# tigrazone/zig_raytracing_contest

Measured on AMD Instinct MI355X. Metric: Mrays/sec + wall-clock to output.png on contest config.json scene, higher is better.
Workload: dtype f32; 1 GPU; cfg3: contest stand-in (99480 tris, 553091 refs), 1920x1080, 256 spp, max_bounce 4, grid 128^3; global_batch=530841600, parallelism=tiles1, schedule=timed: default pass sets

## Files before the change

### include/zrt.h

```cpp
#ifndef ZRT_H
#define ZRT_H

#include <stddef.h>
#include <stdint.h>

#ifdef __cplusplus
extern "C" {
#endif

#define ZRT_ABI_VERSION 2

typedef enum zrt_status {
    ZRT_OK = 0,
    ZRT_ERR_INVALID_ARG = -1,
    ZRT_ERR_NO_DEVICE = -2,
    ZRT_ERR_HIP = -3,
    ZRT_ERR_OUT_OF_MEMORY = -4,
    ZRT_ERR_UNSUPPORTED = -5,
    ZRT_ERR_IO = -6,
    ZRT_ERR_PARSE = -7,
    ZRT_ERR_NOT_FOUND = -8,
    ZRT_ERR_CAMERA = -9,
} zrt_status;

// ... 46 lines not shown
    uint64_t seed;
    int32_t device;
    uint32_t rank;
    uint32_t num_ranks;
    uint32_t tile_size;
    uint32_t flags;
    uint32_t samples_per_pass;
    uint32_t num_devices;
    uint32_t _reserved0;
    const int32_t* devices;
} zrt_render_config;

#define ZRT_FLAG_COUNT_STATS  0x1u
#define ZRT_FLAG_LANE_WALK    0x2u
#define ZRT_FLAG_ONE_SET      0x10u
#define ZRT_FLAG_KERNEL_TIMES 0x20u
#define ZRT_FLAG_ESCAPE       0x40u
#define ZRT_FLAG_NO_ESCAPE    0x80u
#define ZRT_FLAG_FRUSTUM      0x100u
#define ZRT_FLAG_NO_FRUSTUM   0x200u
#define ZRT_FLAG_MT_EXACT     0x400u
#define ZRT_FLAG_RELEASE      0x800u
#define ZRT_FLAG_NO_RELEASE   0x1000u

typedef struct zrt_stats {
    uint64_t segments;
    uint64_t cells_visited;
    uint64_t triangle_tests;
    uint64_t hits;
    uint64_t samples;
    double render_ms;
    double trace_kernel_ms;
    uint32_t trace_launches;
    uint32_t _pad;
} zrt_stats;

const char* zrt_error_string(int status);
int zrt_abi_version(void);
int zrt_device_count(int* count);
int zrt_device_warmup(int device);

typedef struct zrt_geometry zrt_geometry;

int zrt_geometry_build(const float* positions, const float* normals, const float* texcoords,
                       const uint32_t* material, uint32_t num_triangles,
                       const uint32_t resolution[3], uint32_t num_threads, zrt_geometry** out);
// ... 120 lines not shown
```

### zig_raytracing_contest_amd/csrc/escape.h

```cpp
#pragma once
#include <stdint.h>

#include "zrt_math.h"

namespace zrt {

#ifndef ZRT_ESC_BINS
#define ZRT_ESC_BINS 8
#endif
constexpr uint32_t kEscBins = ZRT_ESC_BINS;
constexpr uint32_t kEscNBin = 6 * kEscBins * kEscBins;
constexpr uint32_t kEscWords = kEscNBin <= 128 ? 4 : (kEscNBin + 31) / 32;
constexpr double kEscEps = 1e-3;

ZHD uint32_t esc_dir_bin(v3 d) {
    const float ax = fabsf(d.x), ay = fabsf(d.y), az = fabsf(d.z);
    uint32_t a;
    float m, u, v;
#if defined(__HIP_DEVICE_COMPILE__)
#define ZRT_ESC_RCP(x) __builtin_amdgcn_rcpf(x)
#else
#define ZRT_ESC_RCP(x) (1.0f / (x))
#endif
    if (ax >= ay && ax >= az) { a = 0; m = d.x; const float r = ZRT_ESC_RCP(ax); u = d.y * r; v = d.z * r; }
// ... 163 lines not shown
            }
            if (first < 0) first = it;
            last = it;
            run = 0;
        } else {
            if (run == 0) gap_it = it;
            ++run;
        }
    }
    frustum_finish(q, first, last, fb);
    if (first >= 0 && best_len > 0.0) {
        const double ta = (best0 * q.ds) * q.dmax, tb = (best1 * q.ds) * q.dmin;
        float ga = (float)ta, gb = (float)tb;
        if ((double)ga < ta) ga = nextafterf(ga, kInf);
        if ((double)gb > tb) gb = nextafterf(gb, 0.0f);
        if (ga < gb) {
            fb.ga = ga;
            fb.gb = gb;
        }
    }
    return fb;
}

}
```

### zig_raytracing_contest_amd/csrc/render.hip

```cpp
#include <hip/hip_runtime.h>

#include <algorithm>
#include <cstdio>
#include <cstdlib>
#include <cstring>
#include <ctime>
#include <new>
#include <vector>

#include "zrt_internal.h"
#include "dda.h"
#include "escape.h"
#include "device_geometry.h"

using namespace zrt;

#define HIP_TRY(expr)                                                            \
    do {                                                                         \
        hipError_t _e = (expr);                                                  \
        if (_e != hipSuccess) {                                                  \
            if (getenv("ZRT_DEBUG"))                                             \
                fprintf(stderr, "zrt: %s failed: %s (%s:%d)\n", #expr,           \
                        hipGetErrorString(_e), __FILE__, __LINE__);              \
            return _e == hipErrorOutOfMemory ? ZRT_ERR_OUT_OF_MEMORY : ZRT_ERR_HIP; \
// ... 489 lines not shown
}

struct WfParams {
    TraceParams t;
    const float4* q_in;
    float4* q_out;
    float4* stk4;
    float2* stk2;
    float4* term;
    uint32_t T;
    uint32_t* fetch8;
    const uint32_t* n_in8;
    uint32_t* n_out8;
    float4* hit;
    uint32_t* fetch8s;
    const uint32_t* occx;
    uint32_t occx_words, occx_nbw, occx_moff, occx_nb0, occx_nb01;
    uint32_t occx_ldsw;
    uint32_t test_min;
    uint32_t refill_min;
    uint32_t rel_min;
    uint32_t rel_emin;
    const uint32_t* esc;
};

constexpr uint32_t kCtr = 32;

__device__ __forceinline__ uint32_t xcd_q0(uint32_t P, uint32_t g) {
    const uint32_t nblk = (P + 63u) >> 6;
    return min(P, (nblk * g / 8u) * 64u);
}

__device__ __forceinline__ uint32_t region_base(const WfParams& w, uint32_t g) { return w.t.S * xcd_q0(w.t.P, g); }

#ifdef ZRT_SWEEP
#define SHADE_STAMP(k, v) do { if (sp) { asm volatile("" :: "v"(v)); const uint64_t t_ = __builtin_amdgcn_s_memtime(); \
    const uint32_t n_ = (uint32_t)__popcll(__ballot(1)); \
    if (first_active_lane()) { sp[k] += t_ - sp[16]; sp[16] = t_; sp[8 + (k)] += n_; } } } while (0)
#else
#define SHADE_STAMP(k, v) do { (void)sp; } while (0)
#endif
struct TriRec {
    float4 d0, d1, d2, d3;
};
__device__ __forceinline__ TriRec tri_rec(const TraceParams& p, float t, uint32_t hidx) {
    TriRec r;
// ... 242 lines not shown
#define ZRT_PARK_CHUNK 256
#endif
constexpr uint32_t kParkChunk = ZRT_PARK_CHUNK;
#ifndef ZRT_PARK_LATE_DRAIN
#define ZRT_PARK_LATE_DRAIN 1
#endif
#ifndef ZRT_PARK_QPF
#define ZRT_PARK_QPF 0
#endif
#ifndef ZRT_PARK_ADAPT
#define ZRT_PARK_ADAPT 1
#endif
__device__ __forceinline__ void park_load_range(const TraceParams& p, uint32_t pc, uint32_t* rng) {
    const uint32_t* c = p.cell32 + 8ull * pc;
    const uint32_t m0 = __builtin_amdgcn_readfirstlane((uint32_t)(uintptr_t)rng);
    asm volatile("s_mov_b32 m0, %2\n\t"
                 "global_load_lds_dword %0, off\n\t"
                 "s_add_u32 m0, m0, 0x100\n\t"
                 "global_load_lds_dword %1, off"
                 :
                 : "v"(c), "v"(c + 1), "s"(m0)
                 : "memory");
}
__device__ __forceinline__ void park_load_cell(const TraceParams& p, uint32_t pc, uint32_t face, uint32_t* rng) {
    const uint32_t* c = p.cell32 + 8ull * pc;
    const uint32_t m0 = __builtin_amdgcn_readfirstlane((uint32_t)(uintptr_t)rng);
    asm volatile("s_mov_b32 m0, %3\n\t"
                 "global_load_lds_dword %0, off\n\t"
                 "s_add_u32 m0, m0, 0x100\n\t"
                 "global_load_lds_dword %1, off\n\t"
                 "s_add_u32 m0, m0, 0x100\n\t"
                 "global_load_lds_dword %2, off"
                 :
                 : "v"(c), "v"(c + 1), "v"(c + 2 + face), "s"(m0)
                 : "memory");
}

__device__ __forceinline__ void park_load_esc(const uint32_t* word, uint32_t* esc) {
    const uint32_t m0 = __builtin_amdgcn_readfirstlane((uint32_t)(uintptr_t)esc);
    asm volatile("s_mov_b32 m0, %1\n\t"
                 "global_load_lds_dword %0, off"
                 :
                 : "v"(word), "s"(m0)
                 : "memory");
}

struct ParkSlot {
    float4 o[64];
    float4 d[64];
    unsigned long long best[64];
    float2 uv[64];
    uint32_t mark[64];
};

__device__ __forceinline__ uint32_t wave_excl_sum(uint32_t x, uint32_t lane, uint32_t& total) {
    uint32_t s = x;
    s += (uint32_t)__builtin_amdgcn_update_dpp(0, (int)s, 0x111, 0xf, 0xf, true);
    s += (uint32_t)__builtin_amdgcn_update_dpp(0, (int)s, 0x112, 0xf, 0xf, true);
// ... 113 lines not shown
                    ce = min(base + chunk, lim);
                    cgrp = grp;
                }
                const uint32_t take = min((uint32_t)__popcll(idle), ce - cb);
                const uint32_t rank = (uint32_t)__popcll(idle & below);
                if (st == kIdle && rank < take) {
                    {
                        qi = ent_index<false>(w, cgrp, cb + rank);
                        {
                            const float4 qa = w.q_in[3ull * qi], qb = w.q_in[3ull * qi + 1];
                            o = mk(qa.x, qa.y, qa.z);
                            d = mk(qb.x, qb.y, qb.z);
                        }
                        {
                            nearest = kInf;
                            hu = hv = 0.0f;
                            hidx = 0;
                            W.o[lane] = make_float4(o.x, o.y, o.z, 0.0f);
                            W.d[lane] = make_float4(d.x, d.y, d.z, 0.0f);
                            Dda s0;
                            if (ZRT_FAST_QUOT ? dda_init_fq(p.bmin, p.bmax, p.res, p.cs, p.ics, p.cs_ok != 0u, o, d, s0)
                                              : dda_init(p.bmin, p.bmax, p.res, p.cs, o, d, s0)) {
                                ddav_from_t<PK_BM>(s0, gk, pk, s);
                                if (ESC) {
                                    const uint32_t bin = esc_dir_bin(d);
                                    eoff = (bin >> 5) * 4u;
                                    emask = w.esc && s0.neg < 8u ? 1u << (bin & 31u) : 0u;
                                    eb = ~0u;
                                    esc_slot[lane] = 0u;
                                }
                                if (occx_cell<PK_BM>(occx_mask(L, occx_brick<PK_BM>(w, s)), s, pk)) {
                                    park_load_range(p, s.pc, rng_slot);
                                    rng_slot[128 + lane] = ~0u;
                                    st = kPark;
                                } else {
                                    st = kWalk;
                                }
                            } else {
                                st = kDone;
                            }
                        }
                    }
                }
                PARK_STAMP(12);
                cb += take;
                loaded = loaded || take != 0u;
                idle = __ballot(st == kIdle);
            }
            if (ZRT_PARK_LATE_DRAIN && !loaded) __builtin_amdgcn_s_waitcnt(0x3f70);
#if ZRT_PARK_QPF
            if (ce > cb) {
                const uint32_t j = min(cb + lane, ce - 1u);
                park_load_esc(reinterpret_cast<const uint32_t*>(w.q_in + 3ull * ent_index<false>(w, cgrp, j)), qpf_slot);
            }
#endif
            PARK_STAMP(0);
// ... 541 lines not shown
        r.q[3ull * i + 1] = make_float4(d.x, d.y, d.z, __uint_as_float(1u));
        rest = !ray_fast(d);
    }
    const uint64_t m = __ballot(rest);
    if (m != 0ull && (threadIdx.x & 63u) == (uint32_t)__builtin_ctzll(m)) atomicAdd(&r.ctr[2], (uint32_t)__popcll(m));
}

__global__ __launch_bounds__(kBlock) void rays_out_kernel(const RayParams r) {
    const uint32_t i = blockIdx.x * kBlock + threadIdx.x;
    if (i >= r.n) return;
    const float4 h = r.w.hit[i];
    ray_store_hit(r.hits, i, h.x, h.y, h.z, __float_as_uint(h.w));
}

using RayFn = void (*)(const RayParams);
const RayFn kRaysWalkBM = (RayFn)rays_walk_kernel<false, true, true, false>;
const RayFn kRaysWalk = (RayFn)rays_walk_kernel<false, true, false, false>;
const RayFn kRaysWalkWide = (RayFn)rays_walk_kernel<false, false, false, false>;
const RayFn kRaysWalkExact = (RayFn)rays_walk_kernel<false, false, false, true>;
const RayFn kRaysWalkCount = (RayFn)rays_walk_kernel<true, false, false, true>;
constexpr uint64_t kTraceChunk = 1ull << 20;
constexpr uint64_t kTraceParkMin = 1ull << 19;
constexpr uint32_t kTraceFlags = ZRT_FLAG_COUNT_STATS | ZRT_FLAG_LANE_WALK | ZRT_FLAG_MT_EXACT | ZRT_FLAG_ESCAPE |
                                 ZRT_FLAG_NO_ESCAPE | ZRT_FLAG_RELEASE | ZRT_FLAG_NO_RELEASE | ZRT_TRACE_PARK;

TraceFn count_fn(uint32_t max_bounce) {
    if (max_bounce <= 4) return (TraceFn)trace_kernel<4>;
    if (max_bounce <= 8) return (TraceFn)trace_kernel<8>;
    if (max_bounce <= 16) return (TraceFn)trace_kernel<16>;
    if (max_bounce <= 32) return (TraceFn)trace_kernel<32>;
    return nullptr;
}

struct DeviceGuard {
    int prev = -1;
    explicit DeviceGuard(int dev) {
        if (hipGetDevice(&prev) != hipSuccess) prev = -1;
        if (dev >= 0) (void)hipSetDevice(dev);
    }
    ~DeviceGuard() {
        if (prev >= 0) (void)hipSetDevice(prev);
    }
};

template <typename T>
int grow(T** p, size_t* cap, size_t n) {
    if (*cap >= n && *p) return ZRT_OK;
// ... 31 lines not shown
    zrt_grid grid{};
    uint32_t ncells = 0, nrefs = 0, nmat = 0;
    uint2* d_cells = nullptr;
    PackK pk{};
    bool packed = false;
    uint32_t* d_cell32 = nullptr;
    float* d_pos = nullptr;
    float4* d_data = nullptr;
    DevMat* d_mats = nullptr;
    float* d_texels = nullptr;
    double* d_zig = nullptr;
    uint32_t* d_occ = nullptr;
    uint32_t occ_shift = 0, occ_nb[3] = {0, 0, 0}, occ_words = 0;
    uint32_t* d_occx = nullptr;
    unsigned long long* d_bmask = nullptr;
    uint32_t* d_esc = nullptr;
    uint32_t* d_sat = nullptr;
    float4* d_tlo = nullptr; size_t tlo_cap = 0;
    bool esc_on = false;
    double rel_frac = 0.0;
    bool rel_on = false;
    bool esc_tried = false;
    double esc_density = 0.0;
    uint32_t occx_words = 0, occx_nbw = 0, occx_moff = 0, occx_nb[3] = {0, 0, 0};
    bool occx_ok = false;
    bool mt_exact = false;
    uint32_t* d_pix = nullptr; size_t pix_cap = 0;
    float4* d_out = nullptr; size_t out_cap = 0;
    struct PassSet {
        hipStream_t stream = nullptr;
        float4* q0 = nullptr; size_t q0_cap = 0;
        float4* q1 = nullptr; size_t q1_cap = 0;
        float4* term = nullptr; size_t term_cap = 0;
        float4* stk4 = nullptr; size_t stk4_cap = 0;
        float2* stk2 = nullptr; size_t stk2_cap = 0;
        uint32_t* wfc = nullptr; size_t wfc_cap = 0;
        float4* hit = nullptr; size_t hit_cap = 0;
        hipEvent_t ev_join = nullptr;
    };
    PassSet set[kMaxPassSets];
    float4* d_acc = nullptr; size_t acc_cap = 0;
    uint8_t* d_rgb = nullptr; size_t rgb_cap = 0;
    float* d_lin = nullptr; size_t lin_cap = 0;
    float* d_rays = nullptr; size_t rays_cap = 0;
    uint32_t* d_hits = nullptr; size_t hits_cap = 0;
    std::vector<hipEvent_t> ev_pass;
// ... 103 lines not shown
    if (hipGetDeviceCount(&n) != hipSuccess || n <= 0) return ZRT_ERR_NO_DEVICE;
    const double t1 = StageClock::now_ms();
    if (device < 0) device = 0;
    if (device >= n) return ZRT_ERR_NO_DEVICE;
    DeviceGuard g(device);
    HIP_TRY(hipFree(nullptr));
    const double t2 = StageClock::now_ms();
    hipFuncAttributes fa;
    HIP_TRY(hipFuncGetAttributes(&fa, (const void*)resolve_kernel));
    const double t3 = StageClock::now_ms();
    const int rc = grid_build_warmup();
    if (timing)
        fprintf(stderr, "timing: warm-up: runtime init (hipGetDeviceCount) %.3f ms, device context %.3f ms, "
                "render.hip code object %.3f ms, grid_build.hip code object %.3f ms\n",
                t1 - t0, t2 - t1, t3 - t2, StageClock::now_ms() - t3);
    return rc;
}

extern "C" void zrt_context_destroy(zrt_context* c) {
    if (!c) return;
    DeviceGuard g(c->device);
    if (c->d_cell32) (void)hipFree(c->d_cell32);
    void* bufs[] = {c->d_cells, c->d_pos, c->d_data, c->d_mats, c->d_texels, c->d_zig, c->d_occ, c->d_occx, c->d_esc,
                    c->d_bmask, c->d_sat, c->d_tlo,
                    c->d_pix, c->d_out, c->d_acc, c->d_rgb, c->d_lin, c->d_rays, c->d_hits, c->d_counter, c->d_stats};
    for (void* b : bufs)
        if (b) (void)hipFree(b);
    for (zrt_context::PassSet& ps : c->set) {
        void* sb[] = {ps.q0, ps.q1, ps.term, ps.stk4, ps.stk2, ps.wfc, ps.hit};
        for (void* b : sb)
            if (b) (void)hipFree(b);
        if (ps.ev_join) (void)hipEventDestroy(ps.ev_join);
        if (ps.stream && ps.stream != c->stream) (void)hipStreamDestroy(ps.stream);
    }
    for (hipEvent_t e : c->ev_trace) (void)hipEventDestroy(e);
    for (hipEvent_t e : c->ev_pass) (void)hipEventDestroy(e);
    for (hipEvent_t e : c->ev_k) (void)hipEventDestroy(e);
    if (c->ev_fork) (void)hipEventDestroy(c->ev_fork);
    if (c->ev_begin) (void)hipEventDestroy(c->ev_begin);
    if (c->ev_end) (void)hipEventDestroy(c->ev_end);
    if (c->stream) (void)hipStreamDestroy(c->stream);
    delete c;
}

namespace {

__global__ __launch_bounds__(kBlock) void occx_mask_kernel(const uint2* __restrict__ cells, uint32_t r0, uint32_t r1,
// ... 136 lines not shown
    if (!pack_is_linear(r, c->pk)) HIP_TRY(hipMemsetAsync(c->d_cell32, 0, 32 * n, c->stream));
    hipLaunchKernelGGL(cell32_kernel, dim3(std::min<uint32_t>((c->ncells + kBlock - 1) / kBlock, 16384)), dim3(kBlock),
                       0, c->stream, c->d_cells, r[0], r[1], r[2], c->ncells, c->pk, c->d_pos,
                       c->d_cell32);
    HIP_TRY(hipGetLastError());
    {
        unsigned long long h[2] = {0, 0};
        unsigned long long* d = nullptr;
        HIP_TRY(hipMalloc((void**)&d, sizeof h));
        hipError_t e = hipMemsetAsync(d, 0, sizeof h, c->stream);
        if (e == hipSuccess) {
            hipLaunchKernelGGL(release_stat_kernel, dim3(std::min<uint64_t>((n + kBlock - 1) / kBlock, 4096)),
                               dim3(kBlock), 0, c->stream, (const uint32_t*)c->d_cell32, n, d);
            e = hipGetLastError();
        }
        if (e == hipSuccess) e = hipMemcpyAsync(h, d, sizeof h, hipMemcpyDeviceToHost, c->stream);
        if (e == hipSuccess) e = hipStreamSynchronize(c->stream);
        (void)hipFree(d);
        HIP_TRY(e);
        c->rel_frac = h[0] ? (double)h[1] / (double)h[0] : 0.0;
        c->rel_on = c->rel_frac >= kRelMinFrac;
    }
    HIP_TRY(hipStreamSynchronize(c->stream));
    return ZRT_OK;
}

static int context_counters(zrt_context* c) {
    StageClock sc;
    int rc = context_packed(c);
    if (rc != ZRT_OK) return rc;
    sc.mark(c, "cell records (cell32_kernel)");
    HIP_TRY(hipMalloc((void**)&c->d_counter, 64));
    HIP_TRY(hipMalloc((void**)&c->d_stats, 512));
    return ZRT_OK;
}

static int context_init(zrt_context* c, const zrt_scene* s) {
    int rc = context_base(c);
    if (rc != ZRT_OK) return rc;
    c->grid = s->grid;
    c->ncells = s->num_cells;
    c->nrefs = s->num_triangles;
    c->nmat = s->num_materials;
    c->mt_exact = needs_mt_exact(s->triangles_pos, 9ull * s->num_triangles, 9u, 3u, 0x1p62f);
    HIP_TRY(hipMalloc((void**)&c->d_cells, 8ull * c->ncells));
    HIP_TRY(copy_sync(c->d_cells, s->cells, 8ull * c->ncells, hipMemcpyHostToDevice, c->stream));
// ... 547 lines not shown
        c->pix.resize(std::max<uint32_t>(n, 1));
        tile_pixels(key[0], key[1], key[2], key[3], key[4], c->pix.data(), &n);
        c->pix.resize(n);
        int r2 = grow(&c->d_pix, &c->pix_cap, std::max<size_t>(n, 1));
        if (r2 != ZRT_OK) return r2;
        if (n) HIP_TRY(copy_sync(c->d_pix, c->pix.data(), n * sizeof(uint32_t), hipMemcpyHostToDevice, c->stream));
        memcpy(c->pix_key, key, sizeof key);
        c->pix_valid = true;
    }
    const uint32_t P = (uint32_t)c->pix.size();
    zrt_stats st{};
    if (P == 0) { if (stats) *stats = st; return ZRT_OK; }

    const uint32_t spp = cfg->num_samples;
    const uint32_t mb = cfg->max_bounce;
    const uint32_t nb = std::max<uint32_t>(mb, 1);
    const uint64_t per_item = counting ? 16ull : 96ull + 16ull + 16ull + (ZRT_PLANES16 ? 32ull : 24ull) * nb;
    const bool big = (uint64_t)P * cfg->num_samples >= kSetsMinSamples;
    uint32_t want_sets = big ? kPassSets : 1u;
#if defined(ZRT_SWEEP) || defined(ZRT_SETS_ENV)
    if (const char* e = getenv("ZRT_SETS")) want_sets = (uint32_t)std::max(1, std::min((int)kMaxPassSets, atoi(e)));
#endif
    const bool ktimes = (cfg->flags & ZRT_FLAG_KERNEL_TIMES) != 0;
    size_t held = 16ull * c->out_cap;
    for (const zrt_context::PassSet& ps : c->set)
        held += 16ull * (ps.q0_cap + ps.q1_cap + ps.term_cap + ps.stk4_cap + ps.hit_cap) + 8ull * ps.stk2_cap +
                4ull * ps.wfc_cap;
    const uint64_t s_pass = pass_samples(cfg, per_item, P, counting ? 1u : want_sets, held, c->mem_share);
    const uint32_t npasses = (uint32_t)((spp + s_pass - 1) / s_pass);
    const uint32_t plan_sets = counting ? 1u : std::min<uint32_t>(npasses, want_sets);
    const uint32_t nsets = (cfg->flags & ZRT_FLAG_ONE_SET) ? 1u : plan_sets;
    uint32_t lead_pct = plan_sets > 1 ? kLeadPct : 0u;
#if defined(ZRT_SWEEP) || defined(ZRT_SETS_ENV)
    if (const char* e = getenv("ZRT_LEAD")) lead_pct = plan_sets > 1 ? (uint32_t)std::max(0, std::min(50, atoi(e))) : 0u;
#endif
    const uint64_t last_n = spp - (uint64_t)(npasses - 1) * s_pass;
    const uint64_t cap_items = std::max<uint64_t>(1, 0x7FFFFF00ull / P);
    const uint32_t lead = npasses > 1 ? (uint32_t)std::min<uint64_t>(
                                            {s_pass * lead_pct / 100, last_n - 1, cap_items - std::min(cap_items, s_pass)})
                                      : 0u;
    auto pass_first = [&](uint32_t pass) -> uint32_t { return pass == 0 ? 0u : (uint32_t)(pass * s_pass + lead); };
    auto pass_count = [&](uint32_t pass) -> uint32_t {
        return pass == 0 ? (uint32_t)std::min<uint64_t>(spp, s_pass + lead)
                         : (uint32_t)std::min<uint64_t>(s_pass, spp - pass_first(pass));
    };
    const uint64_t T = (s_pass + lead) * P;
    int rc;
// ... 44 lines not shown
    const bool park_next = c->occx_ok && !counting && !(cfg->flags & ZRT_FLAG_LANE_WALK) &&
                           c->packed && !mtx;
    const bool rel = !(cfg->flags & ZRT_FLAG_NO_RELEASE) && (c->rel_on || (cfg->flags & ZRT_FLAG_RELEASE));
    uint32_t test_min = rel ? kParkTestMinRel : kParkTestMin, refill_min = kParkRefillMin;
#if defined(ZRT_SWEEP) || defined(ZRT_SETS_ENV)
    if (const char* e = getenv("ZRT_PARK_T")) test_min = (uint32_t)std::max(1, std::min(64, atoi(e)));
    if (const char* e = getenv("ZRT_PARK_R")) refill_min = (uint32_t)std::max(1, std::min(64, atoi(e)));
#endif
    uint32_t rel_min = test_min;
    uint32_t rel_emin = 1;
#if defined(ZRT_SWEEP) || defined(ZRT_SETS_ENV)
    if (const char* e = getenv("ZRT_PARK_REL")) rel_min = (uint32_t)std::max(1, std::min(64, atoi(e)));
    if (const char* e = getenv("ZRT_PARK_REL_E")) rel_emin = (uint32_t)std::max(1, std::min(64, atoi(e)));
#endif
    const bool packed = c->packed && !mtx;
    const bool pbm = packed && c->pk.bm;
    const WfFn f_first = mtx ? kWfPrimaryExact : packed ? (pbm ? kWfPrimaryBM : kWfPrimary) : kWfPrimaryWide;
    if (!c->esc_tried && park_next && !(cfg->flags & ZRT_FLAG_NO_ESCAPE) && (big || (cfg->flags & ZRT_FLAG_ESCAPE))) {
        c->esc_tried = true;
        if ((rc = context_escape(c)) != ZRT_OK) return rc;
    }
    const bool esc = c->d_esc && !(cfg->flags & ZRT_FLAG_NO_ESCAPE) &&
                     (c->esc_on || (cfg->flags & ZRT_FLAG_ESCAPE));
    const WfFn f_next = park_next ? (pbm ? (esc ? (WfFn)wf_park_kernel<true, true> : (WfFn)wf_park_kernel<false, true>)
                                         : (esc ? (WfFn)wf_park_kernel<true, false> : (WfFn)wf_park_kernel<false, false>))
                                  : mtx ? kWfBounceExact : (packed ? (pbm ? kWfBounceBM : kWfBounce) : kWfBounceWide);
    const WfFn s_next = c->nmat <= kLdsMats ? (WfFn)wf_shade_kernel<true> : (WfFn)wf_shade_kernel<false>;
    const WfFn s_last = !ZRT_SHADE_LAST ? s_next
                        : c->nmat <= kLdsMats ? (WfFn)wf_shade_kernel<true, true> : (WfFn)wf_shade_kernel<false, true>;
    const size_t lds_shade = c->nmat <= kLdsMats ? c->nmat * sizeof(DevMat) : 0;
    for (uint32_t k = 0; k < nsets && park_next; ++k)
        if ((rc = grow(&c->set[k].hit, &c->set[k].hit_cap, T)) != ZRT_OK) return rc;

    {
        auto shortfall = [&](const char* what, const void* ptr, size_t cap, uint64_t need) {
            if (ptr && cap >= need) return false;
            if (getenv("ZRT_DEBUG"))
                fprintf(stderr, "zrt: capacity guard: %s holds %zu, the launch writes %llu\n", what, ptr ? cap : 0,
                        (unsigned long long)need);
            return true;
        };
        bool bad = shortfall("pixel list", c->d_pix, c->pix_cap, P) || shortfall("rgb", c->d_rgb, c->rgb_cap, 3ull * P) ||
                   (npasses > 1 && shortfall("accumulator", c->d_acc, c->acc_cap, P)) ||
                   (want_lin && shortfall("linear", c->d_lin, c->lin_cap, 3ull * P)) ||
                   (counting && shortfall("counting output", c->d_out, c->out_cap, T));
        for (uint32_t k = 0; k < nsets && !counting && !bad; ++k) {
// ... 133 lines not shown
        tp.sdiv = div_magic(S);
        const int first = pass == 0 ? 1 : 0, last = pass + 1 == npasses ? 1 : 0;
        if (!counting) {
            HIP_TRY(hipMemsetAsync(wfc, 0, 4ull * 32 * kCtr * (mb + 2), sm));
            WfParams W;
            memset(&W, 0, sizeof W);
            W.t = tp;
            W.stk4 = stk4;
            W.stk2 = stk2;
            W.term = term;
            W.T = (uint32_t)T;
            W.occx = c->d_occx;
            W.occx_words = c->occx_words;
            W.occx_ldsw = occx_ldsw;
            W.occx_nbw = c->occx_nbw;
            W.occx_moff = c->occx_moff;
            W.occx_nb0 = c->occx_nb[0];
            W.occx_nb01 = c->occx_nb[0] * c->occx_nb[1];
            W.test_min = test_min;
            W.refill_min = refill_min;
            W.rel_min = rel ? rel_min : 0u;
            W.rel_emin = rel_emin;
            W.esc = c->d_esc;
            for (uint32_t k = 0; k < nb; ++k) {
                W.q_in = (k & 1) ? q0 : q1;
                W.q_out = (k & 1) ? q1 : q0;
                W.fetch8 = wfc + kCtr * (16 * k);
                W.n_in8 = wfc + kCtr * (16 * k + 8);
                W.n_out8 = wfc + kCtr * (16 * (k + 1) + 8);
                W.hit = hit;
                W.fetch8s = wfc + kCtr * (16 * (mb + 2) + 8 * k);
                HIP_TRY(hipEventRecord(c->ev_trace[ne++], sm));
                const int cls = k == 0 ? ZRT_KERNEL_PRIMARY : (park_next ? ZRT_KERNEL_PARK : ZRT_KERNEL_BOUNCE);
                if ((rc = kt_begin(cls, sm)) != ZRT_OK) return rc;
                if (k == 0)
                    hipLaunchKernelGGL(f_first, dim3(grid_first), dim3(thr_first), lds_first, sm, W);
                else
                    hipLaunchKernelGGL(f_next, dim3(grid_next), dim3(thr_next), lds_next, sm, W);
                HIP_TRY(hipGetLastError());
                if ((rc = kt_end(sm)) != ZRT_OK) return rc;
                ++kp.launches[cls];
                if (k > 0 && park_next) {
                    if ((rc = kt_begin(ZRT_KERNEL_SHADE, sm)) != ZRT_OK) return rc;
                    if (k + 1 == nb)
                        hipLaunchKernelGGL(s_last, dim3(grid_shade_last), dim3(kTraceThreads), lds_shade, sm, W);
                    else
// ... 133 lines not shown

extern "C" int zrt_context_trace(zrt_context* c, const zrt_ray_batch* b, zrt_stats* stats) {
    if (!c || !b) return ZRT_ERR_INVALID_ARG;
    if ((b->flags & ~kTraceFlags) != 0u || b->on_device > 1u) return ZRT_ERR_INVALID_ARG;
    zrt_stats st{};
    if (b->num_rays == 0) { if (stats) *stats = st; return ZRT_OK; }
    if (!b->rays || !b->hits) return ZRT_ERR_INVALID_ARG;
    DeviceGuard g(c->device);

    const bool counting = (b->flags & ZRT_FLAG_COUNT_STATS) != 0;
    const bool mtx = c->mt_exact || (b->flags & ZRT_FLAG_MT_EXACT);
    const bool park_ok = c->occx_ok && !counting && !(b->flags & ZRT_FLAG_LANE_WALK) && c->packed && !mtx;
    const bool park = park_ok && ((b->flags & ZRT_TRACE_PARK) || b->num_rays >= kTraceParkMin);
    const bool packed = c->packed && !mtx;
    const bool pbm = packed && c->pk.bm;
    const bool rel = !(b->flags & ZRT_FLAG_NO_RELEASE) && (c->rel_on || (b->flags & ZRT_FLAG_RELEASE));
    int rc;
    if (!c->esc_tried && park && !(b->flags & ZRT_FLAG_NO_ESCAPE) &&
        (b->num_rays >= kSetsMinSamples || (b->flags & ZRT_FLAG_ESCAPE))) {
        c->esc_tried = true;
        if ((rc = context_escape(c)) != ZRT_OK) return rc;
    }
    const bool esc = c->d_esc && !(b->flags & ZRT_FLAG_NO_ESCAPE) && (c->esc_on || (b->flags & ZRT_FLAG_ESCAPE));
    const RayFn f_fast = (counting || mtx) ? nullptr : packed ? (pbm ? kRaysWalkBM : kRaysWalk) : kRaysWalkWide;
    const RayFn f_exact = counting ? kRaysWalkCount : kRaysWalkExact;
    const WfFn f_park = pbm ? (esc ? (WfFn)wf_park_kernel<true, true> : (WfFn)wf_park_kernel<false, true>)
                            : (esc ? (WfFn)wf_park_kernel<true, false> : (WfFn)wf_park_kernel<false, false>);

    zrt_context::PassSet& ps = c->set[0];
    const uint64_t per_ray = (b->on_device ? 0ull : 40ull) + (park ? 64ull : 0ull);
    const size_t held = 4ull * (c->rays_cap + c->hits_cap) + 16ull * (ps.q0_cap + ps.hit_cap);
    size_t budget = (size_t)144 << 30;
    size_t free_b = 0, total_b = 0;
    if (hipMemGetInfo(&free_b, &total_b) == hipSuccess && free_b) budget = std::min(budget, (free_b + held) / 10 * 6);
    budget /= std::max<uint32_t>(c->mem_share, 1u);
    uint64_t chunk = std::min<uint64_t>(kTraceChunk, b->num_rays);
    if (per_ray) chunk = std::max<uint64_t>(64, std::min<uint64_t>(chunk, budget / per_ray));
    if (!b->on_device) {
        if ((rc = grow(&c->d_rays, &c->rays_cap, 6 * chunk)) != ZRT_OK) return rc;
        if ((rc = grow(&c->d_hits, &c->hits_cap, 4 * chunk)) != ZRT_OK) return rc;
    }
    const size_t wfc_words = 32ull * kCtr * 2;
    if (park) {
        if ((rc = grow(&ps.q0, &ps.q0_cap, 3 * chunk)) != ZRT_OK) return rc;
        if ((rc = grow(&ps.hit, &ps.hit_cap, chunk)) != ZRT_OK) return rc;
        if ((rc = grow(&ps.wfc, &ps.wfc_cap, wfc_words)) != ZRT_OK) return rc;
    }
    if ((!b->on_device && (!c->d_rays || c->rays_cap < 6 * chunk || !c->d_hits || c->hits_cap < 4 * chunk)) ||
        (park && (!ps.q0 || ps.q0_cap < 3 * chunk || !ps.hit || ps.hit_cap < chunk || !ps.wfc ||
                  ps.wfc_cap < wfc_words)))
        return ZRT_ERR_INVALID_ARG;
    while (c->ev_trace.size() < 2) {
        hipEvent_t e;
        HIP_TRY(hipEventCreate(&e));
// ... 13 lines not shown
    memset(&R, 0, sizeof R);
    scene_params(c, R.w.t);
    R.w.t.max_bounce = 1;
    R.w.t.counter = c->d_counter;
    R.w.t.stats = c->d_stats;
    R.ctr = c->d_counter;
    if (park) {
        R.w.q_in = ps.q0;
        R.w.hit = ps.hit;
        R.w.fetch8 = ps.wfc;
        R.w.n_in8 = ps.wfc + 8 * kCtr;
        R.w.occx = c->d_occx;
        R.w.occx_words = c->occx_words;
        R.w.occx_ldsw = occx_ldsw;
        R.w.occx_nbw = c->occx_nbw;
        R.w.occx_moff = c->occx_moff;
        R.w.occx_nb0 = c->occx_nb[0];
        R.w.occx_nb01 = c->occx_nb[0] * c->occx_nb[1];
        R.w.test_min = rel ? kParkTestMinRel : kParkTestMin;
        R.w.refill_min = kParkRefillMin;
        R.w.rel_min = rel ? R.w.test_min : 0u;
        R.w.rel_emin = 1;
        R.w.esc = c->d_esc;
        R.q = ps.q0;
        R.n_in8 = ps.wfc + 8 * kCtr;
    }

    HIP_TRY(hipMemsetAsync(c->d_stats, 0, 512, c->stream));
    HIP_TRY(hipEventRecord(c->ev_begin, c->stream));
    uint32_t launches = 0;
    for (uint64_t off = 0; off < b->num_rays; off += chunk) {
        const uint32_t n = (uint32_t)std::min<uint64_t>(chunk, b->num_rays - off);
        if (b->on_device) {
            R.rays = b->rays + 6 * off;
            R.hits = reinterpret_cast<uint32_t*>(b->hits + off);
        } else {
            HIP_TRY(hipMemcpyAsync(c->d_rays, b->rays + 6 * off, 24ull * n, hipMemcpyHostToDevice, c->stream));
            R.rays = c->d_rays;
            R.hits = c->d_hits;
            HIP_TRY(hipEventRecord(c->ev_trace[0], c->stream));
        }
        R.n = n;
        HIP_TRY(hipMemsetAsync(c->d_counter, 0, 64, c->stream));
        const uint32_t nblk = (n + kBlock - 1) / kBlock;
        if (park) {
            HIP_TRY(hipMemsetAsync(ps.wfc, 0, 4ull * 16 * kCtr, c->stream));
// ... 209 lines not shown
            break;
        }
        case ZRT_PROBE_QUOT: {
            const float* a = (const float*)in + 2ull * i;
            float* o = (float*)out + 2ull * i;
            o[0] = quot_rn(a[0], a[1], mt_inv_det<false>(a[1]));
            o[1] = a[0] / a[1];
            break;
        }
        case ZRT_PROBE_RECIP: {
            const float x = ((const float*)in)[i];
            float* o = (float*)out + 2ull * i;
            o[0] = mt_inv_det<false>(x);
            o[1] = mt_inv_det<true>(x);
            break;
        }
        default:
            break;
    }
}

__global__ __launch_bounds__(kBlock) void recip_sweep_kernel(uint32_t lo, uint32_t count, uint32_t* out) {
    uint32_t bad = 0, first = 0xFFFFFFFFu;
    for (uint32_t k = blockIdx.x * kBlock + threadIdx.x; k < count; k += gridDim.x * kBlock) {
        const float x = __uint_as_float(lo + k);
        const float a = mt_inv_det<false>(x), b = mt_inv_det<true>(x);
        const bool same = __float_as_uint(a) == __float_as_uint(b) || (a != a && b != b);
        if (!same) { ++bad; first = min(first, lo + k); }
    }
    for (int o = 32; o > 0; o >>= 1) {
        bad += __shfl_xor(bad, o);
        first = min(first, (uint32_t)__shfl_xor(first, o));
    }
    if ((threadIdx.x & 63u) == 0 && bad) {
        atomicAdd(&out[0], bad);
        atomicMin(&out[1], first);
    }
}

__global__ __launch_bounds__(kBlock) void quot_sweep_kernel(uint32_t s0, uint32_t ns, uint32_t* out) {
    const uint64_t total = (uint64_t)ns << 23;
    uint32_t bad = 0;
    unsigned long long first = ~0ull;
    for (uint64_t k = (uint64_t)blockIdx.x * kBlock + threadIdx.x; k < total; k += (uint64_t)gridDim.x * kBlock) {
        const uint32_t ab = 0x3F800000u | (uint32_t)(k & 0x7FFFFFu);
        const uint32_t bb = 0x3F800000u | (s0 + (uint32_t)(k >> 23));
        const float a = __uint_as_float(ab), b = __uint_as_float(bb);
        const float q = quot_rn(a, b, mt_inv_det<false>(b));
        if (__float_as_uint(q) != __float_as_uint(a / b)) {
            ++bad;
            first = min(first, ((unsigned long long)bb << 32) | ab);
// ... 106 lines not shown
```

### zig_raytracing_contest_amd/native.py

```python
from __future__ import annotations

import ctypes as C
import os

import numpy as np

_HERE = os.path.dirname(os.path.abspath(__file__))
LIB_PATH = os.environ.get("ZRT_LIB") or os.path.join(_HERE, "libzrt.so")
_lib = None

ZRT_OK = 0
STATUS = {0: "ok", -1: "invalid argument", -2: "no HIP device", -3: "HIP runtime error",
          -4: "out of memory", -5: "unsupported configuration", -6: "I/O error",
          -7: "parse error", -8: "not found", -9: "camera/output size rules violated"}
FLAG_COUNT_STATS, FLAG_LANE_WALK = 0x1, 0x2
FLAG_ESCAPE, FLAG_NO_ESCAPE = 0x40, 0x80
FLAG_FRUSTUM, FLAG_NO_FRUSTUM = 0x100, 0x200
FLAG_ONE_SET, FLAG_KERNEL_TIMES = 0x10, 0x20
FLAG_MT_EXACT = 0x400
FLAG_RELEASE, FLAG_NO_RELEASE = 0x800, 0x1000
TRACE_PARK = 0x10000
MISS = 0xFFFFFFFF
KERNEL_CLASSES = ("primary", "park", "shade", "bounce", "resolve", "count")

PROBE_TRIANGLE, PROBE_BBOX, PROBE_DDA, PROBE_TO_RGB = 0, 1, 2, 3
PROBE_RNG_F32, PROBE_RNG_NORM, PROBE_EXP_LOG, PROBE_TEXTURE = 4, 5, 6, 7
PROBE_TRIANGLE_FLAT = 8
PROBE_RECIP, PROBE_RECIP_SWEEP, PROBE_TRIANGLE_EXACT = 9, 10, 11
PROBE_QUOT, PROBE_QUOT_SWEEP = 12, 13
DDA_PROBE_WIDTH = 4 + 4 * 64


class ZrtError(RuntimeError):
    def __init__(self, status, what=""):
        self.status = status
        super().__init__(f"{what}: {STATUS.get(status, status)} ({status})")


class Grid(C.Structure):
    _fields_ = [("bbox_min", C.c_float * 3), ("bbox_max", C.c_float * 3),
                ("resolution", C.c_uint32 * 3), ("cell_size", C.c_float * 3)]


# ... 479 lines not shown
```

Before: 7147 Mrays/s.

## Add per-cell, per-direction-bin backface cull masks for parked triangle tests

Builds a table of 32-bit masks per packed cell and coarse direction bin that clears triangles whose back faces every ray in the bin would see, using a conservative double-precision test over the bin's corner directions. The park path loads this mask instead of the all-ones mask, so it skips intersection tests for those triangles. The table is built once after a statistics pass and is enabled only if enough bits clear per word. The cost is extra device memory, a one-time build, and a dependency on one-sided hit semantics.

```diff
diff --git a/include/zrt.h b/include/zrt.h
--- a/include/zrt.h
+++ b/include/zrt.h
@@ -92,6 +92,8 @@
 #define ZRT_FLAG_MT_EXACT     0x400u
 #define ZRT_FLAG_RELEASE      0x800u
 #define ZRT_FLAG_NO_RELEASE   0x1000u
+#define ZRT_FLAG_BFCULL       0x2000u
+#define ZRT_FLAG_NO_BFCULL    0x4000u
 
 typedef struct zrt_stats {
     uint64_t segments;
diff --git a/zig_raytracing_contest_amd/csrc/escape.h b/zig_raytracing_contest_amd/csrc/escape.h
--- a/zig_raytracing_contest_amd/csrc/escape.h
+++ b/zig_raytracing_contest_amd/csrc/escape.h
@@ -209,4 +209,44 @@
     return fb;
 }
 
-}
+#ifndef ZRT_BFC_BINS
+#define ZRT_BFC_BINS 4
+#endif
+constexpr uint32_t kBfcBins = ZRT_BFC_BINS;
+static_assert(kBfcBins >= 1 && kEscBins % kBfcBins == 0, "a cull bin is a union of escape bins");
+constexpr uint32_t kBfcNBin = 6 * kBfcBins * kBfcBins;
+constexpr double kBfcMargin = 0x1p-21;
+
+ZHD uint32_t bfc_bin_of(uint32_t esc_bin) {
+    constexpr uint32_t q = kEscBins / kBfcBins;
+    const uint32_t f = esc_bin / (kEscBins * kEscBins), iu = (esc_bin / kEscBins) % kEscBins, iv = esc_bin % kEscBins;
+    return (f * kBfcBins + iu / q) * kBfcBins + iv / q;
+}
+ZHD bool bfc_dir_ok(v3 d) {
+    const float s = (fabsf(d.x) + fabsf(d.y)) + fabsf(d.z);
+    return s >= 1e-30f && s <= 4.0f;
+}
+ZHD bool bfc_cull(const float e1[3], const float e2[3], uint32_t bin, double margin = kBfcMargin,
+                  double eps = kEscEps) {
+    for (int k = 0; k < 3; ++k)
+        if (!(fabsf(e1[k]) < kInf) || !(fabsf(e2[k]) < kInf)) return false;
+    const uint32_t fc = bin / (kBfcBins * kBfcBins), iu = (bin / kBfcBins) % kBfcBins, iv = bin % kBfcBins;
+    const int a = (int)(fc / 2u), b = a == 0 ? 1 : 0, c = a == 2 ? 1 : 2;
+    const double nb = (double)kBfcBins;
+    const double uu[2] = {-1.0 + 2.0 * iu / nb - eps, -1.0 + 2.0 * (iu + 1) / nb + eps};
+    const double vv[2] = {-1.0 + 2.0 * iv / nb - eps, -1.0 + 2.0 * (iv + 1) / nb + eps};
+    const double ax = e1[0], ay = e1[1], az = e1[2], bx = e2[0], by = e2[1], bz = e2[2];
+    for (int k = 0; k < 4; ++k) {
+        double D[3];
+        D[a] = (fc & 1u) ? -1.0 : 1.0;
+        D[b] = uu[k & 1];
+        D[c] = vv[k >> 1];
+        const double det = ax * (D[1] * bz - D[2] * by) + ay * (D[2] * bx - D[0] * bz) + az * (D[0] * by - D[1] * bx);
+        const double S = fabs(ax) * (fabs(D[1] * bz) + fabs(D[2] * by)) + fabs(ay) * (fabs(D[2] * bx) + fabs(D[0] * bz)) +
+                         fabs(az) * (fabs(D[0] * by) + fabs(D[1] * bx));
+        if (!(S <= 0x1p120) || !(det + margin * S < 0.0)) return false;
+    }
+    return true;
+}
+
+}
diff --git a/zig_raytracing_contest_amd/csrc/render.hip b/zig_raytracing_contest_amd/csrc/render.hip
--- a/zig_raytracing_contest_amd/csrc/render.hip
+++ b/zig_raytracing_contest_amd/csrc/render.hip
@@ -535,6 +535,8 @@
     uint32_t rel_min;
     uint32_t rel_emin;
     const uint32_t* esc;
+    const uint32_t* bfc;
+    uint64_t bfc_ones;
 };
 
 constexpr uint32_t kCtr = 32;
@@ -823,7 +825,8 @@
                  : "v"(c), "v"(c + 1), "s"(m0)
                  : "memory");
 }
-__device__ __forceinline__ void park_load_cell(const TraceParams& p, uint32_t pc, uint32_t face, uint32_t* rng) {
+__device__ __forceinline__ void park_load_masked(const TraceParams& p, uint32_t pc, const uint32_t* mask,
+                                                 uint32_t* rng) {
     const uint32_t* c = p.cell32 + 8ull * pc;
     const uint32_t m0 = __builtin_amdgcn_readfirstlane((uint32_t)(uintptr_t)rng);
     asm volatile("s_mov_b32 m0, %3\n\t"
@@ -833,8 +836,11 @@
                  "s_add_u32 m0, m0, 0x100\n\t"
                  "global_load_lds_dword %2, off"
                  :
-                 : "v"(c), "v"(c + 1), "v"(c + 2 + face), "s"(m0)
+                 : "v"(c), "v"(c + 1), "v"(mask), "s"(m0)
                  : "memory");
+}
+__device__ __forceinline__ void park_load_cell(const TraceParams& p, uint32_t pc, uint32_t face, uint32_t* rng) {
+    park_load_masked(p, pc, p.cell32 + 8ull * pc + 2 + face, rng);
 }
 
 __device__ __forceinline__ void park_load_esc(const uint32_t* word, uint32_t* esc) {
@@ -994,16 +1000,22 @@
                             if (ZRT_FAST_QUOT ? dda_init_fq(p.bmin, p.bmax, p.res, p.cs, p.ics, p.cs_ok != 0u, o, d, s0)
                                               : dda_init(p.bmin, p.bmax, p.res, p.cs, o, d, s0)) {
                                 ddav_from_t<PK_BM>(s0, gk, pk, s);
+                                const uint32_t bin = (ESC || w.bfc) ? esc_dir_bin(d) : 0u;
                                 if (ESC) {
-                                    const uint32_t bin = esc_dir_bin(d);
                                     eoff = (bin >> 5) * 4u;
                                     emask = w.esc && s0.neg < 8u ? 1u << (bin & 31u) : 0u;
                                     eb = ~0u;
                                     esc_slot[lane] = 0u;
                                 }
                                 if (occx_cell<PK_BM>(occx_mask(L, occx_brick<PK_BM>(w, s)), s, pk)) {
-                                    park_load_range(p, s.pc, rng_slot);
-                                    rng_slot[128 + lane] = ~0u;
+                                    if (w.bfc) {
+                                        const uint64_t wi = bfc_dir_ok(d) ? (uint64_t)s.pc * kBfcNBin + bfc_bin_of(bin)
+                                                                          : w.bfc_ones;
+                                        park_load_masked(p, s.pc, w.bfc + wi, rng_slot);
+                                    } else {
+                                        park_load_range(p, s.pc, rng_slot);
+                                        rng_slot[128 + lane] = ~0u;
+                                    }
                                     st = kPark;
                                 } else {
                                     st = kWalk;
@@ -1591,7 +1603,8 @@
 constexpr uint64_t kTraceChunk = 1ull << 20;
 constexpr uint64_t kTraceParkMin = 1ull << 19;
 constexpr uint32_t kTraceFlags = ZRT_FLAG_COUNT_STATS | ZRT_FLAG_LANE_WALK | ZRT_FLAG_MT_EXACT | ZRT_FLAG_ESCAPE |
-                                 ZRT_FLAG_NO_ESCAPE | ZRT_FLAG_RELEASE | ZRT_FLAG_NO_RELEASE | ZRT_TRACE_PARK;
+                                 ZRT_FLAG_NO_ESCAPE | ZRT_FLAG_RELEASE | ZRT_FLAG_NO_RELEASE | ZRT_FLAG_BFCULL |
+                                 ZRT_FLAG_NO_BFCULL | ZRT_TRACE_PARK;
 
 TraceFn count_fn(uint32_t max_bounce) {
     if (max_bounce <= 4) return (TraceFn)trace_kernel<4>;
@@ -1669,6 +1682,13 @@
     bool rel_on = false;
     bool esc_tried = false;
     double esc_density = 0.0;
+    uint32_t* d_bfc = nullptr;
+    size_t bfc_bytes = 0;
+    bool bfc_tried = false, bfc_tried_forced = false;
+    bool bfc_stat = false;
+    bool bfc_on = false;
+    double bfc_frac = 0.0;
+    double bfc_cleared = 0.0;
     uint32_t occx_words = 0, occx_nbw = 0, occx_moff = 0, occx_nb[3] = {0, 0, 0};
     bool occx_ok = false;
     bool mt_exact = false;
@@ -1818,7 +1838,7 @@
     DeviceGuard g(c->device);
     if (c->d_cell32) (void)hipFree(c->d_cell32);
     void* bufs[] = {c->d_cells, c->d_pos, c->d_data, c->d_mats, c->d_texels, c->d_zig, c->d_occ, c->d_occx, c->d_esc,
-                    c->d_bmask, c->d_sat, c->d_tlo,
+                    c->d_bfc, c->d_bmask, c->d_sat, c->d_tlo,
                     c->d_pix, c->d_out, c->d_acc, c->d_rgb, c->d_lin, c->d_rays, c->d_hits, c->d_counter, c->d_stats};
     for (void* b : bufs)
         if (b) (void)hipFree(b);
@@ -2001,6 +2021,105 @@
         c->rel_on = c->rel_frac >= kRelMinFrac;
     }
     HIP_TRY(hipStreamSynchronize(c->stream));
+    return ZRT_OK;
+}
+
+__global__ __launch_bounds__(kBlock) void bfc_build_kernel(const uint32_t* __restrict__ rec, uint64_t ncell,
+                                                           const float* __restrict__ pos, uint32_t* __restrict__ out,
+                                                           unsigned long long* __restrict__ stat) {
+    const uint64_t total = ncell * kBfcNBin;
+    unsigned long long bits = 0, cleared = 0, words = 0, empty = 0;
+    for (uint64_t i = (uint64_t)blockIdx.x * kBlock + threadIdx.x; i < total; i += (uint64_t)gridDim.x * kBlock) {
+        const uint64_t pc = i / kBfcNBin;
+        const uint32_t bin = (uint32_t)(i - pc * kBfcNBin);
+        const uint32_t b = rec[8 * pc], n = rec[8 * pc + 1] - b;
+        uint32_t m = ~0u;
+        if (n >= 1u && n <= 32u) {
+            for (uint32_t r = 0; r < n; ++r) {
+                float e1[3], e2[3];
+                for (uint32_t k = 0; k < 3; ++k) {
+                    e1[k] = __uint_as_float(tri_word(pos, b + r, 3 + k));
+                    e2[k] = __uint_as_float(tri_word(pos, b + r, 6 + k));
+                }
+                if (bfc_cull(e1, e2, bin)) m &= ~(1u << r);
+            }
+            const uint32_t all = n == 32u ? ~0u : (1u << n) - 1u;
+            bits += n;
+            cleared += n - (uint32_t)__popc(m & all);
+            words += 1;
+            empty += (m & all) == 0u ? 1 : 0;
+        }
+        if (out) out[i] = m;
+    }
+    if (out && blockIdx.x == 0 && threadIdx.x == 0) out[total] = ~0u;
+    bits = wave_sum(bits);
+    cleared = wave_sum(cleared);
+    words = wave_sum(words);
+    empty = wave_sum(empty);
+    if ((threadIdx.x & 63u) == 0) {
+        atomicAdd(&stat[0], bits);
+        atomicAdd(&stat[1], cleared);
+        atomicAdd(&stat[2], words);
+        atomicAdd(&stat[3], empty);
+    }
+}
+
+#ifndef ZRT_BFC_BUDGET_MB
+#define ZRT_BFC_BUDGET_MB 2048
+#endif
+constexpr uint64_t kBfcBudget = (uint64_t)ZRT_BFC_BUDGET_MB << 20;
+#ifndef ZRT_BFC_MIN_CLEARED
+#define ZRT_BFC_MIN_CLEARED 1.0
+#endif
+constexpr double kBfcMinCleared = ZRT_BFC_MIN_CLEARED;
+static int context_bfcull(zrt_context* c, bool forced) {
+    if (c->d_bfc || !c->packed || !c->d_cell32) return ZRT_OK;
+    const uint64_t n = 1ull << (c->pk.b0 + c->pk.b1 + c->pk.b2);
+    const uint64_t bytes = 4ull * (n * kBfcNBin + 1);
+    if (bytes > kBfcBudget / std::max<uint32_t>(c->mem_share, 1u)) return ZRT_OK;
+    size_t free_b = 0, total_b = 0;
+    if (hipMemGetInfo(&free_b, &total_b) != hipSuccess || free_b / 4 < bytes) return ZRT_OK;
+    unsigned long long* d = nullptr;
+    HIP_TRY(hipMalloc((void**)&d, 4 * sizeof(unsigned long long)));
+    const uint64_t blocks = (n * kBfcNBin + kBlock - 1) / kBlock;
+    auto pass = [&](uint32_t* out, unsigned long long* h) -> hipError_t {
+        hipError_t e = hipMemsetAsync(d, 0, 4 * sizeof(unsigned long long), c->stream);
+        if (e != hipSuccess) return e;
+        hipLaunchKernelGGL(bfc_build_kernel, dim3((uint32_t)std::min<uint64_t>(blocks, 1u << 16)), dim3(kBlock), 0,
+                           c->stream, (const uint32_t*)c->d_cell32, n, (const float*)c->d_pos, out, d);
+        if ((e = hipGetLastError()) != hipSuccess) return e;
+        if ((e = hipMemcpyAsync(h, d, 4 * sizeof(unsigned long long), hipMemcpyDeviceToHost, c->stream)) != hipSuccess)
+            return e;
+        return hipStreamSynchronize(c->stream);
+    };
+    unsigned long long h[4] = {0, 0, 0, 0};
+    hipError_t e = hipSuccess;
+    if (!c->bfc_stat) {
+        e = pass(nullptr, h);
+        if (e == hipSuccess) {
+            c->bfc_stat = true;
+            c->bfc_frac = h[0] ? (double)h[1] / (double)h[0] : 0.0;
+            c->bfc_cleared = h[2] ? (double)h[1] / (double)h[2] : 0.0;
+            c->bfc_on = c->bfc_cleared >= kBfcMinCleared;
+            if (getenv("ZRT_WF_DEBUG"))
+                fprintf(stderr, "{\"zrt_bfcull\": {\"bytes\": %llu, \"bins\": %u, \"cleared_frac\": %.4f, "
+                        "\"cleared_per_word\": %.4f, \"empty_word_frac\": %.4f, \"on\": %d}}\n",
+                        (unsigned long long)bytes, kBfcNBin, c->bfc_frac, c->bfc_cleared,
+                        h[2] ? (double)h[3] / (double)h[2] : 0.0, c->bfc_on ? 1 : 0);
+        }
+    }
+    uint32_t* tab = nullptr;
+    if (e == hipSuccess && (c->bfc_on || forced)) {
+        e = hipMalloc((void**)&tab, bytes);
+        if (e == hipSuccess) e = pass(tab, h);
+        if (e != hipSuccess && tab) (void)hipFree(tab);
+    }
+    (void)hipFree(d);
+    HIP_TRY(e);
+    if (tab) {
+        c->d_bfc = tab;
+        c->bfc_bytes = bytes;
+    }
     return ZRT_OK;
 }
 
@@ -2594,7 +2713,7 @@
     if (const char* e = getenv("ZRT_SETS")) want_sets = (uint32_t)std::max(1, std::min((int)kMaxPassSets, atoi(e)));
 #endif
     const bool ktimes = (cfg->flags & ZRT_FLAG_KERNEL_TIMES) != 0;
-    size_t held = 16ull * c->out_cap;
+    size_t held = 16ull * c->out_cap + c->bfc_bytes;
     for (const zrt_context::PassSet& ps : c->set)
         held += 16ull * (ps.q0_cap + ps.q1_cap + ps.term_cap + ps.stk4_cap + ps.hit_cap) + 8ull * ps.stk2_cap +
                 4ull * ps.wfc_cap;
@@ -2685,6 +2804,15 @@
     }
     const bool esc = c->d_esc && !(cfg->flags & ZRT_FLAG_NO_ESCAPE) &&
                      (c->esc_on || (cfg->flags & ZRT_FLAG_ESCAPE));
+    if (park_next && !(cfg->flags & ZRT_FLAG_NO_BFCULL)) {
+        const bool forced = (cfg->flags & ZRT_FLAG_BFCULL) != 0;
+        if (forced ? !c->bfc_tried_forced : (big && !c->bfc_tried)) {
+            c->bfc_tried = true;
+            c->bfc_tried_forced = c->bfc_tried_forced || forced;
+            if ((rc = context_bfcull(c, forced)) != ZRT_OK) return rc;
+        }
+    }
+    const bool bfc = c->d_bfc && !(cfg->flags & ZRT_FLAG_NO_BFCULL) && (c->bfc_on || (cfg->flags & ZRT_FLAG_BFCULL));
     const WfFn f_next = park_next ? (pbm ? (esc ? (WfFn)wf_park_kernel<true, true> : (WfFn)wf_park_kernel<false, true>)
                                          : (esc ? (WfFn)wf_park_kernel<true, false> : (WfFn)wf_park_kernel<false, false>))
                                   : mtx ? kWfBounceExact : (packed ? (pbm ? kWfBounceBM : kWfBounce) : kWfBounceWide);
@@ -2864,6 +2992,8 @@
             W.rel_min = rel ? rel_min : 0u;
             W.rel_emin = rel_emin;
             W.esc = c->d_esc;
+            W.bfc = bfc ? c->d_bfc : nullptr;
+            W.bfc_ones = c->bfc_bytes ? c->bfc_bytes / 4 - 1 : 0;
             for (uint32_t k = 0; k < nb; ++k) {
                 W.q_in = (k & 1) ? q0 : q1;
                 W.q_out = (k & 1) ? q1 : q0;
@@ -3043,6 +3173,15 @@
         if ((rc = context_escape(c)) != ZRT_OK) return rc;
     }
     const bool esc = c->d_esc && !(b->flags & ZRT_FLAG_NO_ESCAPE) && (c->esc_on || (b->flags & ZRT_FLAG_ESCAPE));
+    if (park && !(b->flags & ZRT_FLAG_NO_BFCULL)) {
+        const bool forced = (b->flags & ZRT_FLAG_BFCULL) != 0;
+        if (forced ? !c->bfc_tried_forced : (b->num_rays >= kSetsMinSamples && !c->bfc_tried)) {
+            c->bfc_tried = true;
+            c->bfc_tried_forced = c->bfc_tried_forced || forced;
+            if ((rc = context_bfcull(c, forced)) != ZRT_OK) return rc;
+        }
+    }
+    const bool bfc = c->d_bfc && !(b->flags & ZRT_FLAG_NO_BFCULL) && (c->bfc_on || (b->flags & ZRT_FLAG_BFCULL));
     const RayFn f_fast = (counting || mtx) ? nullptr : packed ? (pbm ? kRaysWalkBM : kRaysWalk) : kRaysWalkWide;
     const RayFn f_exact = counting ? kRaysWalkCount : kRaysWalkExact;
     const WfFn f_park = pbm ? (esc ? (WfFn)wf_park_kernel<true, true> : (WfFn)wf_park_kernel<false, true>)
@@ -3050,7 +3189,7 @@
 
     zrt_context::PassSet& ps = c->set[0];
     const uint64_t per_ray = (b->on_device ? 0ull : 40ull) + (park ? 64ull : 0ull);
-    const size_t held = 4ull * (c->rays_cap + c->hits_cap) + 16ull * (ps.q0_cap + ps.hit_cap);
+    const size_t held = 4ull * (c->rays_cap + c->hits_cap) + 16ull * (ps.q0_cap + ps.hit_cap) + c->bfc_bytes;
     size_t budget = (size_t)144 << 30;
     size_t free_b = 0, total_b = 0;
     if (hipMemGetInfo(&free_b, &total_b) == hipSuccess && free_b) budget = std::min(budget, (free_b + held) / 10 * 6);
@@ -3110,6 +3249,8 @@
         R.w.rel_min = rel ? R.w.test_min : 0u;
         R.w.rel_emin = 1;
         R.w.esc = c->d_esc;
+        R.w.bfc = bfc ? c->d_bfc : nullptr;
+        R.w.bfc_ones = c->bfc_bytes ? c->bfc_bytes / 4 - 1 : 0;
         R.q = ps.q0;
         R.n_in8 = ps.wfc + 8 * kCtr;
     }
@@ -3365,11 +3506,11 @@
 
 __global__ __launch_bounds__(kBlock) void recip_sweep_kernel(uint32_t lo, uint32_t count, uint32_t* out) {
     uint32_t bad = 0, first = 0xFFFFFFFFu;
-    for (uint32_t k = blockIdx.x * kBlock + threadIdx.x; k < count; k += gridDim.x * kBlock) {
-        const float x = __uint_as_float(lo + k);
+    for (uint64_t k = (uint64_t)blockIdx.x * kBlock + threadIdx.x; k < count; k += (uint64_t)gridDim.x * kBlock) {
+        const float x = __uint_as_float(lo + (uint32_t)k);
         const float a = mt_inv_det<false>(x), b = mt_inv_det<true>(x);
         const bool same = __float_as_uint(a) == __float_as_uint(b) || (a != a && b != b);
-        if (!same) { ++bad; first = min(first, lo + k); }
+        if (!same) { ++bad; first = min(first, lo + (uint32_t)k); }
     }
     for (int o = 32; o > 0; o >>= 1) {
         bad += __shfl_xor(bad, o);
diff --git a/zig_raytracing_contest_amd/native.py b/zig_raytracing_contest_amd/native.py
--- a/zig_raytracing_contest_amd/native.py
+++ b/zig_raytracing_contest_amd/native.py
@@ -19,6 +19,7 @@
 FLAG_ONE_SET, FLAG_KERNEL_TIMES = 0x10, 0x20
 FLAG_MT_EXACT = 0x400
 FLAG_RELEASE, FLAG_NO_RELEASE = 0x800, 0x1000
+FLAG_BFCULL, FLAG_NO_BFCULL = 0x2000, 0x4000
 TRACE_PARK = 0x10000
 MISS = 0xFFFFFFFF
 KERNEL_CLASSES = ("primary", "park", "shade", "bounce", "resolve", "count")
```

Result: faster. 7242 Mrays/s, median of 6 (+1.3%).
